# yukw777/EILEV

Hardware: AMD Instinct MI355X
Metric: clips/sec (8-frame, 16 in-context) encode+generate, eilev-blip2-opt-2.7b (higher is better)
Workload: dtype bf16

## Files before the change

### eilev_amd/csrc/gemm_pp4.h

```cpp
#pragma once
#include "gemm_common.h"

namespace {

#ifndef EILEV_PP4_DEEP
#define EILEV_PP4_DEEP 1
#endif
template <int EPI, bool F8 = false, int LN = 0, int M16K = 0, bool A3 = false>
__global__ __launch_bounds__(512, 2) void gemm_pp4_kernel(const GemmArgs g) {
    constexpr bool M16 = M16K != 0, HT16 = M16K == 2;
    static_assert(!M16 || !F8, "16 x 16 form: bf16 instances");
    constexpr int BM = 256, BN = 256, NWM = 2, NWN = 4, NW = 8;
    constexpr int WM = BM / NWM, WN = BN / NWN, TM = WM / 32, TN = WN / 32;
    constexpr int STEP = (BM + BN) * 128;
    constexpr int PC = 8;
    static_assert(!A3 || M16, "A3: lean epilogues only");
    constexpr int STG0 = A3 ? 2 * BM * 128 : 2 * STEP;

    extern __shared__ __attribute__((aligned(16))) char smem[];
    auto a_slot = [&](int st) { return smem + (A3 ? (st % 3) * (BM * 128) : (st & 1) * STEP); };
    auto w_slot = [&](int st) { return smem + (A3 ? 3 * (BM * 128) + (st & 1) * (BN * 128) : (st & 1) * STEP + BM * 128); };
    const int tiles_m = (g.M + BM - 1) / BM, tiles_n = (g.N + BN - 1) / BN, ntiles = tiles_m * tiles_n;
    const int tid = threadIdx.x, lane = tid & 63;
    const int wid = __builtin_amdgcn_readfirstlane(tid >> 6);
    const int wm = wid / NWN, wn = wid % NWN;
    const int l31 = lane & 31, hi = lane >> 5;
    const int l15 = lane & 15, g4 = lane >> 4;
    constexpr int TM16 = WM / 16, TN16 = WN / 16;
    const int ns = g.K / 64;
    const bool late = wid >= NW / 2;
    const int prow = lane >> 3, pslot = lane & 7;

    __amdgpu_buffer_rsrc_t ra = __builtin_amdgcn_make_buffer_rsrc((void *)g.A, 0, 0x7fffffff, 0x00020000);
    const __amdgpu_buffer_rsrc_t rw = __builtin_amdgcn_make_buffer_rsrc((void *)g.W, 0, 0x7fffffff, 0x00020000);
    unsigned po[PC];
    const int pw = late ? wid - NW / 2 : wid;
    auto set_tile = [&](int t, int &m0, int &n0) {
        int tm_i, tn_i;
        tile_coords(g, tiles_m, tiles_n, tm_i, tn_i, t);
        m0 = tm_i * BM;
        n0 = tn_i * BN;
        {
#ifdef EILEV_PP4_PROBE_A0
            const uint64_t base = (uint64_t)(g.A);
#else
            const uint64_t base = (uint64_t)(g.A + (int64_t)m0 * g.lda);
#endif
            const uint64_t ub = ((uint64_t)(unsigned)__builtin_amdgcn_readfirstlane((int)(base >> 32)) << 32) |
                                (unsigned)__builtin_amdgcn_readfirstlane((int)(unsigned)base);
            ra = __builtin_amdgcn_make_buffer_rsrc((void *)ub, 0, 0x7fffffff, 0x00020000);
        }
#pragma unroll
        for (int i = 0; i < PC; ++i) {
            const int row = (pw * PC + i) * 8 + prow;
            const unsigned sw = (unsigned)((pslot ^ ((row >> 1) & 7)) << 4);
            if (!late) {
                int gr = m0 + row;
                gr = gr < g.M ? gr : g.M - 1;
                po[i] = (unsigned)(gr - m0) * (unsigned)(g.lda * 2) + sw;
            } else {
                int gr = n0 + row;
                gr = gr < g.N ? gr : g.N - 1;
                po[i] = (unsigned)gr * (unsigned)(g.ldw * 2) + sw;
            }
        }
    };
    auto stage_step = [&](int st, bool mine = true, int part = 0) {
        char *sd = (late ? w_slot(st) : a_slot(st)) + (pw * PC) * 1024;
        if (!mine) return;
#ifndef EILEV_PP4_PROBE_SKIP
#define EILEV_PP4_PROBE_SKIP 0
#endif
        constexpr int PCE = (EILEV_PP4_PROBE_SKIP & 4) ? 0 : (EILEV_PP4_PROBE_SKIP & 1) ? PC / 2 : PC;
        constexpr int PCL = (EILEV_PP4_PROBE_SKIP & 8) ? 0 : (EILEV_PP4_PROBE_SKIP & 2) ? PC / 2 : PC;
        if (late) {
#pragma unroll
            for (int i = 0; i < PCL; ++i)
                if (part == 0 || (part == 1) == (i < PC / 2)) __builtin_amdgcn_raw_ptr_buffer_load_lds(rw, (lds_void *)(sd + i * 1024), 16, po[i], st * 128, 0, 0);
        } else {
#pragma unroll
            for (int i = 0; i < PCE; ++i)
                if (part == 0 || (part == 1) == (i < PC / 2)) __builtin_amdgcn_raw_ptr_buffer_load_lds(ra, (lds_void *)(sd + i * 1024), 16, po[i], st * 128, 0, 0);
        }
    };
    f32x16 acc[M16 ? 1 : TM][M16 ? 1 : TN];
    bf16x8 af[2][TM], bfr[2][TN];
    typedef __attribute__((ext_vector_type(4))) float f32x4_t;
    f32x4_t acc16[M16 ? TM16 : 1][M16 ? TN16 : 1];
    auto read_half = [&](int st, int h) {
        const char *sa = a_slot(st) + (wm * WM) * 128;
        const char *sb = w_slot(st) + (wn * WN) * 128;
        if constexpr (M16) {
            const int kc = h * 4 + g4;
#pragma unroll
            for (int j = 0; j < TN16; ++j) {
                const int row = j * 16 + l15;
                bfr[j >> 1][j & 1] = *reinterpret_cast<const bf16x8 *>(sb + row * 128 + swz(row, kc));
            }
#pragma unroll
            for (int i = 0; i < TM16; ++i) {
                const int row = i * 16 + l15;
                af[i >> 2][i & 3] = *reinterpret_cast<const bf16x8 *>(sa + row * 128 + swz(row, kc));
            }
            return;
        }
#pragma unroll
        for (int k2 = 0; k2 < 2; ++k2) {
            const int kc = h * 4 + k2 * 2 + hi;
#pragma unroll
            for (int j = 0; j < TN; ++j) {
                const int row = j * 32 + l31;
                bfr[k2][j] = *reinterpret_cast<const bf16x8 *>(sb + row * 128 + swz(row, kc));
            }
#pragma unroll
            for (int i = 0; i < TM; ++i) {
                const int row = i * 32 + l31;
                af[k2][i] = *reinterpret_cast<const bf16x8 *>(sa + row * 128 + swz(row, kc));
            }
        }
    };
    typedef int i32x8_t __attribute__((ext_vector_type(8)));
    struct Pair16 { bf16x8 lo, hi; };
    auto cat32 = [](const bf16x8 &lo, const bf16x8 &hi2) { return __builtin_bit_cast(i32x8_t, Pair16{lo, hi2}); };
    auto mma_half = [&]() {
        __builtin_amdgcn_s_setprio(1);
        if constexpr (F8) {
#pragma unroll
            for (int i = 0; i < TM; ++i)
#pragma unroll
                for (int j = 0; j < TN; ++j)
                    acc[i][j] = __builtin_amdgcn_mfma_scale_f32_32x32x64_f8f6f4(cat32(bfr[0][j], bfr[1][j]), cat32(af[0][i], af[1][i]), acc[i][j],
                                                                               0, 0, 0, 0, 0, 0);
        } else if constexpr (M16) {
#pragma unroll
            for (int i = 0; i < TM16; ++i)
#pragma unroll
                for (int j = 0; j < TN16; ++j)
                    acc16[i][j] = __builtin_amdgcn_mfma_f32_16x16x32_bf16(bfr[j >> 1][j & 1], af[i >> 2][i & 3], acc16[i][j], 0, 0, 0);
        } else {
#pragma unroll
            for (int k2 = 0; k2 < 2; ++k2)
#pragma unroll
                for (int i = 0; i < TM; ++i)
#pragma unroll
                    for (int j = 0; j < TN; ++j)
                        acc[i][j] = __builtin_amdgcn_mfma_f32_32x32x16_bf16(bfr[k2][j], af[k2][i], acc[i][j], 0, 0, 0);
        }
        __builtin_amdgcn_s_setprio(0);
    };
    const int hm = wm * 2 + (wn >> 1), hn = wn & 1;
    auto read_half_ht = [&](int st, int h) {
        const char *sa = a_slot(st) + (hm * 64) * 128;
        const char *sb = w_slot(st) + (hn * 64) * 128;
        if constexpr (M16) {
            const int kc = h * 4 + g4;
#pragma unroll
            for (int j = 0; j < 4; ++j) {
                const int row = j * 16 + l15;
                bfr[j >> 1][j & 1] = *reinterpret_cast<const bf16x8 *>(sb + row * 128 + swz(row, kc));
            }
#pragma unroll
            for (int i = 0; i < 4; ++i) {
                const int row = i * 16 + l15;
                af[0][i] = *reinterpret_cast<const bf16x8 *>(sa + row * 128 + swz(row, kc));
            }
            return;
        }
#pragma unroll
        for (int k2 = 0; k2 < 2; ++k2) {
            const int kc = h * 4 + k2 * 2 + hi;
#pragma unroll
            for (int j = 0; j < 2; ++j) {
                const int row = j * 32 + l31;
                bfr[k2][j] = *reinterpret_cast<const bf16x8 *>(sb + row * 128 + swz(row, kc));
            }
#pragma unroll
            for (int i = 0; i < 2; ++i) {
                const int row = i * 32 + l31;
                af[k2][i] = *reinterpret_cast<const bf16x8 *>(sa + row * 128 + swz(row, kc));
            }
        }
    };
    auto mma_half_ht = [&]() {
        __builtin_amdgcn_s_setprio(1);
        if constexpr (F8) {
#pragma unroll
            for (int i = 0; i < 2; ++i)
#pragma unroll
                for (int j = 0; j < 2; ++j)
                    acc[i][j] = __builtin_amdgcn_mfma_scale_f32_32x32x64_f8f6f4(cat32(bfr[0][j], bfr[1][j]), cat32(af[0][i], af[1][i]), acc[i][j],
                                                                               0, 0, 0, 0, 0, 0);
        } else if constexpr (M16) {
#pragma unroll
            for (int i = 0; i < 4; ++i)
#pragma unroll
                for (int j = 0; j < 4; ++j)
                    acc16[i][j] = __builtin_amdgcn_mfma_f32_16x16x32_bf16(bfr[j >> 1][j & 1], af[0][i], acc16[i][j], 0, 0, 0);
        } else {
#pragma unroll
            for (int k2 = 0; k2 < 2; ++k2)
#pragma unroll
                for (int i = 0; i < 2; ++i)
#pragma unroll
                    for (int j = 0; j < 2; ++j)
                        acc[i][j] = __builtin_amdgcn_mfma_f32_32x32x16_bf16(bfr[k2][j], af[k2][i], acc[i][j], 0, 0, 0);
        }
        __builtin_amdgcn_s_setprio(0);
    };
    char *const stg = smem + STG0 + wid * 4096;
    const unsigned stg_sw = (unsigned)(STG0 + wid * 4096 + l31 * 128 + hi * 8) ^ (unsigned)((l31 & 7) << 4);
    const unsigned stg_sw16 = (unsigned)(STG0 + wid * 4096 + l15 * 128 + (g4 & 1) * 8) ^ (unsigned)((((g4 >> 1) ^ (l15 & 7)) << 4));
    const int srow = lane >> 3, schunk = lane & 7;
    auto is_lean = [&](int n0_) {
        return !(n0_ + 128 >= g.N && !(g.dbg & DBG_GEMM_NO_HALF_TILES)) && n0_ + BN <= g.N && !g.out_f32 && g.patch_group == 0 && g.scale_cols == 0 && !g.wscale && !g.ascale &&
               !(g.dbg & (DBG_GEMM_NO_EPILOGUE | DBG_GEMM_NO_STORES | DBG_GEMM_ROW0_STORES)) && !(g.dbg & DBG_GEMM_PP4_NO_PRESTAGE);
    };
    float ln_rs[LN == 1 ? (M16 ? TM16 : TM) : 1];
    auto lean_epilogue = [&](int cm0, int cn0, auto res_c, auto ht_c) {
        constexpr bool RES = decltype(res_c)::value;
        constexpr bool HTE = decltype(ht_c)::value;
        constexpr int NU = HTE ? 2 : TM;
        const int roff = HTE ? hm * 64 : wm * WM, coff = HTE ? hn * 64 : wn * WN;
        if constexpr (M16K == 1) {
            if (cn0 + coff >= g.N) return;
        }
        constexpr bool LNC = LN == 1 && !RES, LNP = LN == 2 && RES;
        typedef __attribute__((ext_vector_type(4))) unsigned u32x4_t;
        const int r0 = cm0 + roff;
        const int rows = g.M - r0 < 0 ? 0 : (g.M - r0 < NU * 32 ? g.M - r0 : NU * 32);
        auto uniform_rsrc = [&](const void *ptr, int bytes) {
            const uint64_t base = (uint64_t)ptr;
            const uint64_t ub = ((uint64_t)(unsigned)__builtin_amdgcn_readfirstlane((int)(base >> 32)) << 32) |
                                (unsigned)__builtin_amdgcn_readfirstlane((int)(unsigned)base);
            return __builtin_amdgcn_make_buffer_rsrc((void *)ub, 0, __builtin_amdgcn_readfirstlane(bytes), 0x00020000);
        };
        const __amdgpu_buffer_rsrc_t rc = uniform_rsrc(reinterpret_cast<bf16 *>(g.C) + (int64_t)r0 * g.ldc + cn0 + coff, rows * (int)(g.ldc * 2));
        const __amdgpu_buffer_rsrc_t rr = uniform_rsrc(RES ? g.resid + (int64_t)r0 * g.ldr + cn0 + coff : g.A, RES ? rows * (int)(g.ldr * 2) : 0);
        const unsigned st_voff = (unsigned)srow * (unsigned)(g.ldc * 2) + schunk * 16, rs_voff = (unsigned)srow * (unsigned)(g.ldr * 2) + schunk * 16;
#ifndef EILEV_HM_AUX
#define EILEV_HM_AUX EILEV_ST_AUX
#endif
        constexpr bool HMI = LN == 1 && !RES && EPI == 0 && M16K == 1;
        const bool hm = HMI && g.hm_tok != 0;
        __amdgpu_buffer_rsrc_t rch = rc;
        unsigned hm_off = 0, hm_off_w = 0;
        int hm_str2 = 0, hm_t = 0;
        if constexpr (HMI) {
            if (hm) {
                const int TOK = g.hm_tok, HD = g.hm_hd, NH = g.hm_heads, D3 = g.N / 3;
                const int n0 = cn0 + coff;
                const int plane = __builtin_amdgcn_readfirstlane(n0 / D3), rr = n0 - plane * D3;
                int2 ent;
                if (rr < NH * 64) {
                    ent.x = (plane * NH + (rr >> 6)) * TOK * HD + schunk * 8;
                    ent.y = 64;
                } else {
                    const int cph = (HD - 64) >> 3, jb = ((rr - NH * 64) >> 3) + schunk, hh = jb / cph;
                    ent.x = (plane * NH + hh) * TOK * HD + TOK * 64 + (jb - hh * cph) * 8;
                    ent.y = HD - 64;
                }
                const int fw = __builtin_amdgcn_readfirstlane(r0 / TOK);
                const int m0 = r0 + srow, f0 = m0 / TOK;
                hm_t = m0 - f0 * TOK;
                hm_str2 = __builtin_amdgcn_readfirstlane(ent.y * 2);
                hm_off = (unsigned)(((f0 - fw) * TOK * g.N + ent.x + hm_t * ent.y) * 2);
                hm_off_w = hm_off + (unsigned)(TOK * g.N * 2) - (unsigned)(TOK * hm_str2);
                const int64_t left = ((int64_t)g.M / TOK - fw) * TOK * g.N * 2;
                rch = uniform_rsrc(reinterpret_cast<bf16 *>(g.C) + (int64_t)fw * TOK * g.N, (int)(unsigned)(left < 0xfffffff0ll ? left : 0xfffffff0ll));
            }
        }
        u32x4_t rv[4];
        auto res_load = [&](int u) {
#pragma unroll
            for (int it = 0; it < 4; ++it) rv[it] = __builtin_amdgcn_raw_buffer_load_b128(rr, rs_voff, (u * 32 + it * 8) * (int)(g.ldr * 2), 0);
        };
        if constexpr (RES) res_load(0);
        bf16x4 biasr[M16 ? 1 : TN][4];
        bf16x4 biasr16[M16 ? TN16 : 1];
        if constexpr (M16) {
#pragma unroll
            for (int j = 0; j < TN16; ++j) {
                if (g.bias) biasr16[j] = *reinterpret_cast<const bf16x4 *>(g.bias + cn0 + coff + j * 16 + g4 * 4);
                else biasr16[j] = (bf16x4){(bf16)0.f, (bf16)0.f, (bf16)0.f, (bf16)0.f};
            }
        } else {
#pragma unroll
        for (int j = 0; j < TN; ++j)
#pragma unroll
            for (int q = 0; q < 4; ++q) {
                if (g.bias) biasr[j][q] = *reinterpret_cast<const bf16x4 *>(g.bias + cn0 + wn * WN + j * 32 + q * 8 + hi * 4);
                else biasr[j][q] = (bf16x4){(bf16)0.f, (bf16)0.f, (bf16)0.f, (bf16)0.f};
            }
        }
        typedef __attribute__((ext_vector_type(2))) float f32x2_t;
        __amdgpu_buffer_rsrc_t rst = rr;
        if constexpr (LNP) rst = uniform_rsrc(g.stat_out + ((int64_t)((cn0 + coff) >> 6) * g.stat_ld + r0) * 2, rows * 8);
        static_for<NU>([&](auto u_c) {
            constexpr int U = decltype(u_c)::value;
            float st1 = 0.0f, st2 = 0.0f;
            bf16x4 rcell[M16 ? 2 : TN][4];
            if constexpr (RES) {
#pragma unroll
                for (int it = 0; it < 4; ++it) {
                    const int row = it * 8 + srow;
                    *reinterpret_cast<u32x4_t *>(stg + row * 128 + ((schunk ^ (row & 7)) << 4)) = rv[it];
                }
                if constexpr (U + 1 < NU) res_load(U + 1);
                if constexpr (M16) {
#pragma unroll
                    for (int ib = 0; ib < 2; ++ib)
#pragma unroll
                        for (int j = 0; j < TN16; ++j) {
                            unsigned ca;
                            asm volatile("v_xor_b32 %0, %1, %2" : "=v"(ca) : "n"(((j * 2) << 4) | (ib << 11)), "v"(stg_sw16));
                            rcell[ib][j] = *reinterpret_cast<const bf16x4 *>(smem + ca);
                        }
                } else {
#pragma unroll
                for (int j = 0; j < TN; ++j)
#pragma unroll
                    for (int q = 0; q < 4; ++q) {
                        unsigned ca;
                        asm volatile("v_xor_b32 %0, %1, %2" : "=v"(ca) : "n"((j * 4 + q) << 4), "v"(stg_sw));
                        rcell[j][q] = *reinterpret_cast<const bf16x4 *>(smem + ca);
                    }
                }
            }
            float st16[2][2] = {{0.0f, 0.0f}, {0.0f, 0.0f}};
            if constexpr (M16) {
#pragma unroll
                for (int ib = 0; ib < 2; ++ib)
#pragma unroll
                    for (int j = 0; j < TN16; ++j) {
                        float v[4];
                        if constexpr (LNC) {
#pragma unroll
                            for (int e = 0; e < 4; ++e) v[e] = fmaf(acc16[2 * U + ib][j][e], ln_rs[2 * U + ib], (float)biasr16[j][e]);
                        } else {
#pragma unroll
                            for (int e = 0; e < 4; ++e) v[e] = acc16[2 * U + ib][j][e] + (float)biasr16[j][e];
                        }
                        if constexpr (LN == 0 && EPI == 0 && !RES) {
                            if (cn0 + coff + j * 16 < g.scale_cols) {
#pragma unroll
                                for (int e = 0; e < 4; ++e) v[e] *= g.scale;
                            }
                        }
                        if constexpr (EPI == 2) {
#pragma unroll
                            for (int e = 0; e < 4; ++e) v[e] = fmaxf(v[e], 0.0f);
                        }
                        if constexpr (EPI == 1) gelu_erf_n<4>(v);
                        if constexpr (RES) {
#pragma unroll
                            for (int e = 0; e < 4; ++e) v[e] += (float)rcell[ib][j][e];
                        }
                        if constexpr (LNP) {
#pragma unroll
                            for (int e = 0; e < 4; ++e) {
                                st16[ib][0] += v[e];
                                st16[ib][1] = fmaf(v[e], v[e], st16[ib][1]);
                            }
                        }
                        unsigned ca;
                        asm volatile("v_xor_b32 %0, %1, %2" : "=v"(ca) : "n"(((j * 2) << 4) | (ib << 11)), "v"(stg_sw16));
                        *reinterpret_cast<bf16x4 *>(smem + ca) = (bf16x4){(bf16)v[0], (bf16)v[1], (bf16)v[2], (bf16)v[3]};
                    }
            } else {
#pragma unroll
            for (int j = 0; j < TN; ++j)
#pragma unroll
                for (int q = 0; q < 4; ++q) {
                    float v[4];
                    if constexpr (LNC) {
#pragma unroll
                        for (int e = 0; e < 4; ++e) v[e] = fmaf(acc[U][j][q * 4 + e], ln_rs[U], (float)biasr[j][q][e]);
                    } else {
#pragma unroll
                        for (int e = 0; e < 4; ++e) v[e] = acc[U][j][q * 4 + e] + (float)biasr[j][q][e];
                    }
                    if constexpr (EPI == 2) {
#pragma unroll
                        for (int e = 0; e < 4; ++e) v[e] = fmaxf(v[e], 0.0f);
                    }
                    if constexpr (EPI == 1) gelu_erf_n<4>(v);
                    if constexpr (RES) {
#pragma unroll
                        for (int e = 0; e < 4; ++e) v[e] += (float)rcell[j][q][e];
                    }
                    if constexpr (LNP) {
#pragma unroll
                        for (int e = 0; e < 4; ++e) {
                            st1 += v[e];
                            st2 = fmaf(v[e], v[e], st2);
                        }
                    }
                    unsigned ca;
                    asm volatile("v_xor_b32 %0, %1, %2" : "=v"(ca) : "n"((j * 4 + q) << 4), "v"(stg_sw));
                    *reinterpret_cast<bf16x4 *>(smem + ca) = (bf16x4){(bf16)v[0], (bf16)v[1], (bf16)v[2], (bf16)v[3]};
                }
            }
            if constexpr (LNP && M16) {
                typedef __attribute__((ext_vector_type(2))) unsigned u32x2_t;
#pragma unroll
                for (int ib = 0; ib < 2; ++ib) {
                    float a1 = st16[ib][0], a2 = st16[ib][1];
                    a1 += __shfl_xor(a1, 16); a2 += __shfl_xor(a2, 16);
                    a1 += __shfl_xor(a1, 32); a2 += __shfl_xor(a2, 32);
                    const f32x2_t t = (f32x2_t){a1, a2};
                    if (g4 == 0) __builtin_amdgcn_raw_buffer_store_b64(__builtin_bit_cast(u32x2_t, t), rst, (U * 32 + ib * 16 + l15) * 8, 0, 0);
                }
            } else if constexpr (LNP) {
                typedef __attribute__((ext_vector_type(2))) unsigned u32x2_t;
                const f32x2_t t = (f32x2_t){st1 + __shfl_xor(st1, 32), st2 + __shfl_xor(st2, 32)};
                if (hi == 0) __builtin_amdgcn_raw_buffer_store_b64(__builtin_bit_cast(u32x2_t, t), rst, (U * 32 + l31) * 8, 0, 0);
            }
            __builtin_amdgcn_sched_barrier(0);
            bf16x8 erb[2];
#pragma unroll
            for (int h2 = 0; h2 < 2; ++h2) {
#pragma unroll
                for (int b = 0; b < 2; ++b) {
                    const int row = (h2 * 2 + b) * 8 + srow;
                    erb[b] = *reinterpret_cast<const bf16x8 *>(stg + row * 128 + ((schunk ^ (row & 7)) << 4));
                }
                if (hm) {
                    if constexpr (HMI) {
#pragma unroll
                        for (int b = 0; b < 2; ++b) {
                            const int RO = U * 32 + (h2 * 2 + b) * 8;
                            const unsigned vo = hm_t + RO >= g.hm_tok ? hm_off_w : hm_off;
                            __builtin_amdgcn_raw_buffer_store_b128(__builtin_bit_cast(u32x4_t, erb[b]), rch, vo, RO * hm_str2, EILEV_HM_AUX);
                        }
                    }
                } else {
#pragma unroll
                for (int b = 0; b < 2; ++b)
                    __builtin_amdgcn_raw_buffer_store_b128(__builtin_bit_cast(u32x4_t, erb[b]), rc, st_voff, (U * 32 + (h2 * 2 + b) * 8) * (int)(g.ldc * 2), EILEV_ST_AUX);
                }
            }
            asm volatile("s_nop 1" ::: "memory");
            __builtin_amdgcn_sched_barrier(0);
        });
    };
#define PP_WAIT_LGKM0() __builtin_amdgcn_s_waitcnt(0xC07F)
#define PP_WAIT_LGKM0_VM0() __builtin_amdgcn_s_waitcnt(0x0070)
#define PP_WAIT_VM0() __builtin_amdgcn_s_waitcnt(0x0F70)
#define PP_BARRIER()                       \
    do {                                   \
        __builtin_amdgcn_sched_barrier(0); \
        __builtin_amdgcn_s_barrier();      \
        __builtin_amdgcn_sched_barrier(0); \
    } while (0)

    int t = blockIdx.x, m0, n0;
    if (t >= ntiles) return;
    set_tile(t, m0, n0);
    auto w_piece_mine = [&](int n0_) { return !(n0_ + 128 >= g.N && !(g.dbg & DBG_GEMM_NO_HALF_TILES)) || wid < NW / 2 + 2; };
    stage_step(0, w_piece_mine(n0));
    bool pre1 = ns > 1 && (A3 || !(g.dbg & DBG_GEMM_PP4_NO_PRESTAGE));
    if (pre1) stage_step(1, w_piece_mine(n0));
    bool lean_cur = M16 || is_lean(n0);
    float ln_nm[LN == 1 ? (M16 ? TM16 : TM) : 1], ln_cl[LN == 1 ? (M16 ? TN16 : TN) : 1];
    auto ln_fetch = [&](int m0_, int n0_) {
        if constexpr (LN == 1 && M16) {
            const bool ht = HT16 && n0_ + 128 >= g.N;
            const int mb = m0_ + (ht ? hm * 64 : wm * WM) + l15, nb = n0_ + (ht ? hn * 64 : wn * WN) + l15;
            const __amdgpu_buffer_rsrc_t rl = __builtin_amdgcn_make_buffer_rsrc((void *)g.ln_rows, 0, g.M * 8, 0x00020000);
            const __amdgpu_buffer_rsrc_t rcs = __builtin_amdgcn_make_buffer_rsrc((void *)g.ln_csum, 0, g.N * 4, 0x00020000);
#pragma unroll
            for (int i = 0; i < TM16; ++i) ln_nm[i] = __builtin_bit_cast(float, __builtin_amdgcn_raw_buffer_load_b32(rl, (mb + i * 16) * 8 + 4, 0, 0));
#pragma unroll
            for (int j = 0; j < TN16; ++j) ln_cl[j] = __builtin_bit_cast(float, __builtin_amdgcn_raw_buffer_load_b32(rcs, (nb + j * 16) * 4, 0, 0));
        } else if constexpr (LN == 1) {
            const bool ht = n0_ + 128 >= g.N && !(g.dbg & DBG_GEMM_NO_HALF_TILES);
            const int mb = m0_ + (ht ? hm * 64 : wm * WM) + l31, nb = n0_ + (ht ? hn * 64 : wn * WN) + l31;
            const __amdgpu_buffer_rsrc_t rl = __builtin_amdgcn_make_buffer_rsrc((void *)g.ln_rows, 0, g.M * 8, 0x00020000);
            const __amdgpu_buffer_rsrc_t rcs = __builtin_amdgcn_make_buffer_rsrc((void *)g.ln_csum, 0, g.N * 4, 0x00020000);
#pragma unroll
            for (int i = 0; i < TM; ++i) ln_nm[i] = __builtin_bit_cast(float, __builtin_amdgcn_raw_buffer_load_b32(rl, (mb + i * 32) * 8 + 4, 0, 0));
#pragma unroll
            for (int j = 0; j < TN; ++j) ln_cl[j] = __builtin_bit_cast(float, __builtin_amdgcn_raw_buffer_load_b32(rcs, (nb + j * 32) * 4, 0, 0));
        }
    };
    ln_fetch(m0, n0);
    int trace_i = 0;
    const bool tracer = g.trace != nullptr && (wid == 0 || wid == NW / 2) && lane == 0;
#ifdef EILEV_PP4_ITRACE
#define ITR(k)                                                                                                              \
    do {                                                                                                                    \
        if (st == EILEV_PP4_ITRACE && tracer) *reinterpret_cast<volatile unsigned long long *>(stg + (k) * 8) = __builtin_amdgcn_s_memtime(); \
    } while (0)
#else
#define ITR(k) do { } while (0)
#endif
    auto stamp = [&](int k, bool core = false) {
#ifdef EILEV_PP4_ITRACE
        return;
#endif
        if (tracer && trace_i < g.trace_tiles)
            g.trace[(((size_t)blockIdx.x * 2 + (late ? 1 : 0)) * g.trace_tiles + trace_i) * 8 + k] =
                core ? __builtin_amdgcn_s_memtime() : __builtin_amdgcn_s_memrealtime();
    };
    for (; t < ntiles; t += gridDim.x) {
        stamp(0);
        stamp(5, true);
        typedef __attribute__((ext_vector_type(4))) short s16x4_t;
        s16x4_t ln_a1[LN == 1 ? (M16 ? TM16 : TM) : 1], ln_w1[LN == 1 ? (M16 ? TN16 : TN) : 1];
        auto acc_prep = [&]() {
            if constexpr (LN == 1 && M16) {
                const bf16 z = (bf16)0.0f;
#pragma unroll
                for (int i = 0; i < TM16; ++i) {
                    const float m = g4 ? 0.0f : ln_nm[i];
                    const bf16 mh = (bf16)m, ml = (bf16)(m - (float)mh);
                    ln_a1[i] = __builtin_bit_cast(s16x4_t, (bf16x4){mh, mh, ml, z});
                }
#pragma unroll
                for (int j = 0; j < TN16; ++j) {
                    const float c = g4 ? 0.0f : ln_cl[j];
                    const bf16 ch = (bf16)c, cl = (bf16)(c - (float)ch);
                    ln_w1[j] = __builtin_bit_cast(s16x4_t, (bf16x4){ch, cl, ch, z});
                }
            } else if constexpr (LN == 1) {
                const bf16 z = (bf16)0.0f;
#pragma unroll
                for (int i = 0; i < TM; ++i) {
                    const float m = hi ? 0.0f : ln_nm[i];
                    const bf16 mh = (bf16)m, ml = (bf16)(m - (float)mh);
                    ln_a1[i] = __builtin_bit_cast(s16x4_t, (bf16x4){mh, mh, ml, z});
                }
#pragma unroll
                for (int j = 0; j < TN; ++j) {
                    const float c = hi ? 0.0f : ln_cl[j];
                    const bf16 ch = (bf16)c, cl = (bf16)(c - (float)ch);
                    ln_w1[j] = __builtin_bit_cast(s16x4_t, (bf16x4){ch, cl, ch, z});
                }
            }
        };
        auto acc_init = [&]() {
            if constexpr (M16) {
                const f32x4_t zero4 = (f32x4_t){0.0f, 0.0f, 0.0f, 0.0f};
#pragma unroll
                for (int i = 0; i < TM16; ++i)
#pragma unroll
                    for (int j = 0; j < TN16; ++j) {
                        if constexpr (LN == 1) acc16[i][j] = __builtin_amdgcn_mfma_f32_16x16x16bf16_1k(ln_w1[j], ln_a1[i], zero4, 0, 0, 0);
                        else acc16[i][j] = zero4;
                    }
            } else if constexpr (LN == 1) {
                f32x16 zero;
#pragma unroll
                for (int r = 0; r < 16; ++r) zero[r] = 0.0f;
#pragma unroll
                for (int i = 0; i < TM; ++i)
#pragma unroll
                    for (int j = 0; j < TN; ++j) acc[i][j] = __builtin_amdgcn_mfma_f32_32x32x8bf16_1k(ln_w1[j], ln_a1[i], zero, 0, 0, 0);
            } else {
#pragma unroll
                for (int i = 0; i < TM; ++i)
#pragma unroll
                    for (int j = 0; j < TN; ++j)
#pragma unroll
                        for (int r = 0; r < 16; ++r) acc[i][j][r] = 0.0f;
            }
        };
        if constexpr (LN != 1) acc_init();
        asm volatile("s_waitcnt vmcnt(0)" ::: "memory");
        PP_BARRIER();
        if (late) PP_BARRIER();
        stamp(1);
        const int nsd = (g.dbg & DBG_GEMM_ONE_KSTEP) ? 1 : ns;
        const bool half_tile = n0 + 128 >= g.N && !(g.dbg & DBG_GEMM_NO_HALF_TILES);
        auto kstep = [&](int st, auto first_c, auto ht_c) {
            constexpr bool FIRST = decltype(first_c)::value;
            constexpr bool HT = decltype(ht_c)::value;
            const bool w_mine = !HT || wid < NW / 2 + 2;
            ITR(0);
            if constexpr (HT) read_half_ht(st, 0); else read_half(st, 0);
#if EILEV_PP4_DEEP
#ifndef EILEV_PP4_SPLIT
#define EILEV_PP4_SPLIT 3
#endif
#ifndef EILEV_PP4_SPLIT_QKV
#define EILEV_PP4_SPLIT_QKV 0
#endif
            constexpr bool SPLIT_OK = !HT && (EILEV_PP4_SPLIT_QKV || !(LN == 1 && EPI == 0));
            constexpr bool SPLIT_E = (EILEV_PP4_SPLIT & 1) && SPLIT_OK, SPLIT_L = (EILEV_PP4_SPLIT & 2) && SPLIT_OK;
            if (!late) {
                if constexpr (A3) {
                    if (st + 2 < ns) stage_step(st + 2, w_mine, SPLIT_E ? 1 : 0);
                } else if (st + 1 < ns && !(FIRST && pre1)) stage_step(st + 1, w_mine, SPLIT_E ? 1 : 0);
            } else if (FIRST && !pre1 && ns > 1) stage_step(1, w_mine);
            else if (SPLIT_L && !FIRST && st + 1 < ns) stage_step(st + 1, w_mine, 2);
#else
            if (st + 1 < ns && !(FIRST && pre1)) stage_step(st + 1, w_mine);
#endif
            if constexpr (FIRST && LN == 1) acc_prep();
            PP_WAIT_LGKM0();
            ITR(1);
            PP_BARRIER();
            ITR(2);
            if constexpr (FIRST && LN == 1) acc_init();
            if constexpr (HT) mma_half_ht(); else mma_half();
            ITR(3);
            PP_BARRIER();
            ITR(4);
            if constexpr (HT) read_half_ht(st, 1); else read_half(st, 1);
#if EILEV_PP4_DEEP
            PP_WAIT_LGKM0();
            if (late) {
                PP_WAIT_VM0();
                if constexpr (!HT) if (st + 2 < ns) stage_step(st + 2, w_mine, SPLIT_L ? 1 : 0);
            } else if (A3) {
                if (SPLIT_E && st + 2 < ns) stage_step(st + 2, w_mine, 2);
            } else if (SPLIT_E && st + 1 < ns && !(FIRST && pre1)) stage_step(st + 1, w_mine, 2);
            ITR(5);
            PP_BARRIER();
            ITR(6);
            if constexpr (HT) {
                if (late && st + 2 < ns) stage_step(st + 2, w_mine);
                mma_half_ht();
            } else mma_half();
            __builtin_amdgcn_sched_barrier(0);
            if constexpr (A3) {
                if (!late) {
                    if (st + 2 < ns) asm volatile("s_waitcnt vmcnt(8)" ::: "memory");
                    else asm volatile("s_waitcnt vmcnt(0)" ::: "memory");
                }
            } else if (!late) asm volatile("s_waitcnt vmcnt(0)" ::: "memory");
            ITR(7);
            PP_BARRIER();
#else
            PP_WAIT_LGKM0_VM0();
            PP_BARRIER();
            if constexpr (HT) mma_half_ht(); else mma_half();
            PP_BARRIER();
#endif
        };
        if (half_tile && M16K != 1) {
            if constexpr (M16K != 1) {
                kstep(0, std::true_type{}, std::true_type{});
                for (int st = 1; st < nsd; ++st) kstep(st, std::false_type{}, std::true_type{});
            }
        } else {
            kstep(0, std::true_type{}, std::false_type{});
            for (int st = 1; st < nsd; ++st) kstep(st, std::false_type{}, std::false_type{});
        }
        stamp(2);
#ifdef EILEV_PP4_ITRACE
        if (tracer && trace_i < g.trace_tiles) {
#pragma unroll
            for (int k = 0; k < 8; ++k)
                g.trace[(((size_t)blockIdx.x * 2 + (late ? 1 : 0)) * g.trace_tiles + trace_i) * 8 + k] = *reinterpret_cast<volatile unsigned long long *>(stg + k * 8);
        }
#endif
        if (!late) PP_BARRIER();
        if constexpr (LN == 1) {
            const __amdgpu_buffer_rsrc_t rl = __builtin_amdgcn_make_buffer_rsrc((void *)g.ln_rows, 0, g.M * 8, 0x00020000);
            if constexpr (M16) {
#pragma unroll
                for (int i = 0; i < TM16; ++i) ln_rs[i] = __builtin_bit_cast(float, __builtin_amdgcn_raw_buffer_load_b32(rl, (m0 + ((HT16 && half_tile) ? hm * 64 : wm * WM) + i * 16 + l15) * 8, 0, 0));
            } else {
#pragma unroll
            for (int u = 0; u < TM; ++u) ln_rs[u] = __builtin_bit_cast(float, __builtin_amdgcn_raw_buffer_load_b32(rl, (m0 + wm * WM + u * 32 + l31) * 8, 0, 0));
            }
        }
        const int cm0 = m0, cn0 = n0, tn = t + gridDim.x;
        const bool lean = lean_cur;
        pre1 = false;
        lean_cur = false;
        if (tn < ntiles) {
            set_tile(tn, m0, n0);
            stage_step(0, w_piece_mine(n0));
            pre1 = lean && ns > 1;
            if (pre1) stage_step(1, w_piece_mine(n0));
            lean_cur = M16 || is_lean(n0);
            ln_fetch(m0, n0);
        }
        stamp(3);
        if (HT16 && half_tile) {
            if constexpr (HT16) {
                if constexpr (LN == 1) lean_epilogue(cm0, cn0, std::false_type{}, std::true_type{});
                else if constexpr (LN == 2) lean_epilogue(cm0, cn0, std::true_type{}, std::true_type{});
                else if (g.resid != nullptr) lean_epilogue(cm0, cn0, std::true_type{}, std::true_type{});
                else lean_epilogue(cm0, cn0, std::false_type{}, std::true_type{});
            }
        } else if (lean || M16) {
            if constexpr (LN == 1) lean_epilogue(cm0, cn0, std::false_type{}, std::false_type{});
            else if constexpr (LN == 2) lean_epilogue(cm0, cn0, std::true_type{}, std::false_type{});
            else if (g.resid != nullptr) lean_epilogue(cm0, cn0, std::true_type{}, std::false_type{});
            else lean_epilogue(cm0, cn0, std::false_type{}, std::false_type{});
        } else if constexpr (!M16) {
            if (half_tile) {
                gemm_epilogue<64, 64, EPI, 0, 2, LN, true>(g, reinterpret_cast<f32x16(&)[2][2]>(acc), smem + STEP, cm0, cn0, hm, hn, wid, lane);
            } else {
                gemm_epilogue<WM, WN, EPI, 0, TM / 2, LN, true>(g, acc, smem + STEP, cm0, cn0, wm, wn, wid, lane);
                gemm_epilogue<WM, WN, EPI, TM / 2, TM, LN, true>(g, acc, smem + STEP, cm0, cn0, wm, wn, wid, lane);
            }
        }
        stamp(4);
        stamp(6, true);
        ++trace_i;
    }
#undef PP_BARRIER
}

constexpr int PP4_SMEM = 2 * 65536 + 8 * 4096;

}
```

Measured before the change: 229.2.

## Prefetch epilogue bias/residual/LN loads early and use partial vmcnt waits in pp4 GEMM

```diff
diff --git a/eilev_amd/csrc/gemm_pp4.h b/eilev_amd/csrc/gemm_pp4.h
--- a/eilev_amd/csrc/gemm_pp4.h
+++ b/eilev_amd/csrc/gemm_pp4.h
@@ -215,14 +215,112 @@
         return !(n0_ + 128 >= g.N && !(g.dbg & DBG_GEMM_NO_HALF_TILES)) && n0_ + BN <= g.N && !g.out_f32 && g.patch_group == 0 && g.scale_cols == 0 && !g.wscale && !g.ascale &&
                !(g.dbg & (DBG_GEMM_NO_EPILOGUE | DBG_GEMM_NO_STORES | DBG_GEMM_ROW0_STORES)) && !(g.dbg & DBG_GEMM_PP4_NO_PRESTAGE);
     };
+    float ln_nm[LN == 1 ? (M16 ? TM16 : TM) : 1], ln_cl[LN == 1 ? (M16 ? TN16 : TN) : 1];
+    int trace_i = 0;
+    const bool tracer = g.trace != nullptr && (wid == 0 || wid == NW / 2) && lane == 0;
+    auto stamp = [&](int k, bool core = false) {
+#ifdef EILEV_PP4_ITRACE
+        return;
+#endif
+        if (tracer && trace_i < g.trace_tiles)
+            g.trace[(((size_t)blockIdx.x * 2 + (late ? 1 : 0)) * g.trace_tiles + trace_i) * 8 + k] =
+                core ? __builtin_amdgcn_s_memtime() : __builtin_amdgcn_s_memrealtime();
+    };
     float ln_rs[LN == 1 ? (M16 ? TM16 : TM) : 1];
-    auto lean_epilogue = [&](int cm0, int cn0, auto res_c, auto ht_c) {
+    typedef __attribute__((ext_vector_type(2))) unsigned u32x2_e;
+    typedef __attribute__((ext_vector_type(4))) unsigned u32x4_e;
+    u32x2_e ep_bias[M16 ? TN16 : 1];
+#ifndef EILEV_PP4_RES_UNITS
+#define EILEV_PP4_RES_UNITS 1
+#endif
+    constexpr int EP_RU = EILEV_PP4_RES_UNITS;
+    static_assert(EP_RU == 1 || EP_RU == 2, "residual units in front of the DMA");
+    u32x4_e ep_rv[M16 ? EP_RU : 1][4];
+    int ep_young = 0;
+#define PP_ASM_LOAD4(op, step, first, d0, d1, d2, d3, voff, rsrc)                                                                              \
+    asm volatile("s_nop 4\n\t" op " %0, %4, %5, 0 offen offset:%6\n\t" op " %1, %4, %5, 0 offen offset:%7\n\t" op " %2, %4, %5, 0 offen offset:%8\n\t" op \
+                 " %3, %4, %5, 0 offen offset:%9"                                                                                             \
+                 : "=&v"(d0), "=&v"(d1), "=&v"(d2), "=&v"(d3)                                                                                 \
+                 : "v"(voff), "s"(rsrc), "n"(first), "n"((first) + (step)), "n"((first) + 2 * (step)), "n"((first) + 3 * (step)))
+#define PP_ASM_LOAD4_B128(d0, d1, d2, d3, voff, rsrc, s0, s1, s2, s3)                                                                              \
+    asm volatile("s_nop 4\n\tbuffer_load_dwordx4 %0, %4, %5, %6 offen\n\tbuffer_load_dwordx4 %1, %4, %5, %7 offen\n\tbuffer_load_dwordx4 %2, %4, %5, %8 " \
+                 "offen\n\tbuffer_load_dwordx4 %3, %4, %5, %9 offen"                                                                                \
+                 : "=&v"(d0), "=&v"(d1), "=&v"(d2), "=&v"(d3)                                                                                     \
+                 : "v"(voff), "s"(rsrc), "s"(s0), "s"(s1), "s"(s2), "s"(s3))
+    auto epi_block = [&](bool ht, int &roff, int &coff) {
+        roff = (HT16 && ht) ? hm * 64 : wm * WM;
+        coff = (HT16 && ht) ? hn * 64 : wn * WN;
+    };
+    auto epi_res = [&]() { return LN == 2 || (LN == 0 && g.resid != nullptr); };
+    auto epi_rr = [&](int cm0, int cn0, bool ht, int nu) {
+        int roff, coff;
+        epi_block(ht, roff, coff);
+        const int r0 = cm0 + roff;
+        const int rows = (g.M - r0 < 0 || !epi_res()) ? 0 : (g.M - r0 < nu * 32 ? g.M - r0 : nu * 32);
+        const uint64_t base = (uint64_t)(g.resid + (int64_t)r0 * g.ldr + cn0 + coff);
+        const uint64_t ub = ((uint64_t)(unsigned)__builtin_amdgcn_readfirstlane((int)(base >> 32)) << 32) | (unsigned)__builtin_amdgcn_readfirstlane((int)(unsigned)base);
+        return __builtin_amdgcn_make_buffer_rsrc((void *)ub, 0, __builtin_amdgcn_readfirstlane(rows * (int)(g.ldr * 2)), 0x00020000);
+    };
+    auto epi_issue = [&](int cm0, int cn0, bool ht) {
+        if constexpr (M16) {
+            int roff, coff;
+            epi_block(ht, roff, coff);
+            if constexpr (LN == 1) {
+                const __amdgpu_buffer_rsrc_t rl = __builtin_amdgcn_make_buffer_rsrc((void *)g.ln_rows, 0, g.M * 8, 0x00020000);
+                const unsigned vo = (unsigned)(cm0 + roff + l15) * 8u;
+                static_assert(TM16 == 8 && TN16 == 4, "the grouped asm loads below");
+                PP_ASM_LOAD4("buffer_load_dword", 128, 0, ln_rs[0], ln_rs[1], ln_rs[2], ln_rs[3], vo, rl);
+                PP_ASM_LOAD4("buffer_load_dword", 128, 512, ln_rs[4], ln_rs[5], ln_rs[6], ln_rs[7], vo, rl);
+            }
+            {
+                const __amdgpu_buffer_rsrc_t rb = __builtin_amdgcn_make_buffer_rsrc((void *)g.bias, 0, g.bias ? g.N * 2 : 0, 0x00020000);
+                const unsigned vo = (unsigned)(cn0 + coff + g4 * 4) * 2u;
+                PP_ASM_LOAD4("buffer_load_dwordx2", 32, 0, ep_bias[0], ep_bias[1], ep_bias[2], ep_bias[3], vo, rb);
+            }
+            if constexpr (LN != 1) {
+                const __amdgpu_buffer_rsrc_t rr = epi_rr(cm0, cn0, ht, (HT16 && ht) ? 2 : TM);
+                const unsigned vo = (unsigned)srow * (unsigned)(g.ldr * 2) + schunk * 16;
+                const int rs8 = 8 * (int)(g.ldr * 2);
+#pragma unroll
+                for (int u = 0; u < EP_RU; ++u) PP_ASM_LOAD4_B128(ep_rv[u][0], ep_rv[u][1], ep_rv[u][2], ep_rv[u][3], vo, rr, (4 * u) * rs8, (4 * u + 1) * rs8, (4 * u + 2) * rs8, (4 * u + 3) * rs8);
+            }
+        }
+    };
+    auto epi_wait = [&]() {
+        if constexpr (M16) {
+            const int ny = __builtin_amdgcn_readfirstlane(ep_young);
+#define PP_EPI_WAIT_ASM "s_cmp_lt_u32 %[ny], 16\n\ts_cbranch_scc1 1f\n\ts_waitcnt vmcnt(16)\n\ts_branch 3f\n1:\n\ts_cmp_lt_u32 %[ny], 8\n\ts_cbranch_scc1 2f\n\ts_waitcnt vmcnt(8)\n\ts_branch 3f\n2:\n\ts_waitcnt vmcnt(0)\n3:"
+            if constexpr (LN == 1) {
+                asm volatile(PP_EPI_WAIT_ASM
+                             : "+v"(ep_bias[0]), "+v"(ep_bias[1]), "+v"(ep_bias[2]), "+v"(ep_bias[3]), "+v"(ln_rs[0]), "+v"(ln_rs[1]), "+v"(ln_rs[2]), "+v"(ln_rs[3]),
+                               "+v"(ln_rs[4]), "+v"(ln_rs[5]), "+v"(ln_rs[6]), "+v"(ln_rs[7])
+                             : [ny] "s"(ny)
+                             : "memory", "scc");
+                asm volatile("" : "+v"(ln_nm[0]), "+v"(ln_nm[1]), "+v"(ln_nm[2]), "+v"(ln_nm[3]), "+v"(ln_nm[4]), "+v"(ln_nm[5]), "+v"(ln_nm[6]), "+v"(ln_nm[7]),
+                                  "+v"(ln_cl[0]), "+v"(ln_cl[1]), "+v"(ln_cl[2]), "+v"(ln_cl[3]));
+            } else if constexpr (EP_RU == 2) {
+                asm volatile(PP_EPI_WAIT_ASM
+                             : "+v"(ep_bias[0]), "+v"(ep_bias[1]), "+v"(ep_bias[2]), "+v"(ep_bias[3]), "+v"(ep_rv[0][0]), "+v"(ep_rv[0][1]), "+v"(ep_rv[0][2]),
+                               "+v"(ep_rv[0][3]), "+v"(ep_rv[EP_RU - 1][0]), "+v"(ep_rv[EP_RU - 1][1]), "+v"(ep_rv[EP_RU - 1][2]), "+v"(ep_rv[EP_RU - 1][3])
+                             : [ny] "s"(ny)
+                             : "memory", "scc");
+            } else {
+                asm volatile(PP_EPI_WAIT_ASM
+                             : "+v"(ep_bias[0]), "+v"(ep_bias[1]), "+v"(ep_bias[2]), "+v"(ep_bias[3]), "+v"(ep_rv[0][0]), "+v"(ep_rv[0][1]), "+v"(ep_rv[0][2]),
+                               "+v"(ep_rv[0][3])
+                             : [ny] "s"(ny)
+                             : "memory", "scc");
+            }
+#undef PP_EPI_WAIT_ASM
+        }
+    };
+    auto lean_epilogue = [&](int cm0, int cn0, auto res_c, auto ht_c) -> int {
         constexpr bool RES = decltype(res_c)::value;
         constexpr bool HTE = decltype(ht_c)::value;
         constexpr int NU = HTE ? 2 : TM;
         const int roff = HTE ? hm * 64 : wm * WM, coff = HTE ? hn * 64 : wn * WN;
         if constexpr (M16K == 1) {
-            if (cn0 + coff >= g.N) return;
+            if (cn0 + coff >= g.N) return 0;
         }
         constexpr bool LNC = LN == 1 && !RES, LNP = LN == 2 && RES;
         typedef __attribute__((ext_vector_type(4))) unsigned u32x4_t;
@@ -248,6 +346,9 @@
         if constexpr (HMI) {
             if (hm) {
                 const int TOK = g.hm_tok, HD = g.hm_hd, NH = g.hm_heads, D3 = g.N / 3;
+                int zero_o = 0;
+                asm volatile("" : "+v"(zero_o));
+                const int schunk = (int)__builtin_amdgcn_mbcnt_hi(~0u, __builtin_amdgcn_mbcnt_lo(~0u, (unsigned)zero_o)) & 7;
                 const int n0 = cn0 + coff;
                 const int plane = __builtin_amdgcn_readfirstlane(n0 / D3), rr = n0 - plane * D3;
                 int2 ent;
@@ -255,7 +356,9 @@
                     ent.x = (plane * NH + (rr >> 6)) * TOK * HD + schunk * 8;
                     ent.y = 64;
                 } else {
-                    const int cph = (HD - 64) >> 3, jb = ((rr - NH * 64) >> 3) + schunk, hh = jb / cph;
+                    const int cph = (HD - 64) >> 3, jb = ((rr - NH * 64) >> 3) + schunk;
+                    const unsigned mg = (unsigned)__builtin_amdgcn_readfirstlane((int)(0xffffffffu / (unsigned)cph + 1u));
+                    const int hh = cph == 1 ? jb : (int)__umulhi((unsigned)jb, mg);
                     ent.x = (plane * NH + hh) * TOK * HD + TOK * 64 + (jb - hh * cph) * 8;
                     ent.y = HD - 64;
                 }
@@ -274,15 +377,12 @@
 #pragma unroll
             for (int it = 0; it < 4; ++it) rv[it] = __builtin_amdgcn_raw_buffer_load_b128(rr, rs_voff, (u * 32 + it * 8) * (int)(g.ldr * 2), 0);
         };
-        if constexpr (RES) res_load(0);
+        if constexpr (RES && !M16) res_load(0);
         bf16x4 biasr[M16 ? 1 : TN][4];
         bf16x4 biasr16[M16 ? TN16 : 1];
         if constexpr (M16) {
 #pragma unroll
-            for (int j = 0; j < TN16; ++j) {
-                if (g.bias) biasr16[j] = *reinterpret_cast<const bf16x4 *>(g.bias + cn0 + coff + j * 16 + g4 * 4);
-                else biasr16[j] = (bf16x4){(bf16)0.f, (bf16)0.f, (bf16)0.f, (bf16)0.f};
-            }
+            for (int j = 0; j < TN16; ++j) biasr16[j] = __builtin_bit_cast(bf16x4, ep_bias[j]);
         } else {
 #pragma unroll
         for (int j = 0; j < TN; ++j)
@@ -303,9 +403,16 @@
 #pragma unroll
                 for (int it = 0; it < 4; ++it) {
                     const int row = it * 8 + srow;
-                    *reinterpret_cast<u32x4_t *>(stg + row * 128 + ((schunk ^ (row & 7)) << 4)) = rv[it];
-                }
-                if constexpr (U + 1 < NU) res_load(U + 1);
+                    if constexpr (M16) *reinterpret_cast<u32x4_t *>(stg + row * 128 + ((schunk ^ (row & 7)) << 4)) = __builtin_bit_cast(u32x4_t, ep_rv[U % EP_RU][it]);
+                    else *reinterpret_cast<u32x4_t *>(stg + row * 128 + ((schunk ^ (row & 7)) << 4)) = rv[it];
+                }
+                if constexpr (M16) {
+                    if constexpr (U + EP_RU < NU) {
+#pragma unroll
+                        for (int it = 0; it < 4; ++it)
+                            ep_rv[U % EP_RU][it] = __builtin_bit_cast(u32x4_e, __builtin_amdgcn_raw_buffer_load_b128(rr, rs_voff, ((U + EP_RU) * 32 + it * 8) * (int)(g.ldr * 2), 0));
+                    }
+                } else if constexpr (U + 1 < NU) res_load(U + 1);
                 if constexpr (M16) {
 #pragma unroll
                     for (int ib = 0; ib < 2; ++ib)
@@ -442,6 +549,7 @@
             asm volatile("s_nop 1" ::: "memory");
             __builtin_amdgcn_sched_barrier(0);
         });
+        return NU * 4 + (LNP && M16 ? NU * 2 : 0) + (RES && M16 ? (NU - EP_RU) * 4 : 0);
     };
 #define PP_WAIT_LGKM0() __builtin_amdgcn_s_waitcnt(0xC07F)
 #define PP_WAIT_LGKM0_VM0() __builtin_amdgcn_s_waitcnt(0x0070)
@@ -457,21 +565,18 @@
     if (t >= ntiles) return;
     set_tile(t, m0, n0);
     auto w_piece_mine = [&](int n0_) { return !(n0_ + 128 >= g.N && !(g.dbg & DBG_GEMM_NO_HALF_TILES)) || wid < NW / 2 + 2; };
-    stage_step(0, w_piece_mine(n0));
     bool pre1 = ns > 1 && (A3 || !(g.dbg & DBG_GEMM_PP4_NO_PRESTAGE));
-    if (pre1) stage_step(1, w_piece_mine(n0));
     bool lean_cur = M16 || is_lean(n0);
-    float ln_nm[LN == 1 ? (M16 ? TM16 : TM) : 1], ln_cl[LN == 1 ? (M16 ? TN16 : TN) : 1];
     auto ln_fetch = [&](int m0_, int n0_) {
         if constexpr (LN == 1 && M16) {
             const bool ht = HT16 && n0_ + 128 >= g.N;
             const int mb = m0_ + (ht ? hm * 64 : wm * WM) + l15, nb = n0_ + (ht ? hn * 64 : wn * WN) + l15;
             const __amdgpu_buffer_rsrc_t rl = __builtin_amdgcn_make_buffer_rsrc((void *)g.ln_rows, 0, g.M * 8, 0x00020000);
             const __amdgpu_buffer_rsrc_t rcs = __builtin_amdgcn_make_buffer_rsrc((void *)g.ln_csum, 0, g.N * 4, 0x00020000);
-#pragma unroll
-            for (int i = 0; i < TM16; ++i) ln_nm[i] = __builtin_bit_cast(float, __builtin_amdgcn_raw_buffer_load_b32(rl, (mb + i * 16) * 8 + 4, 0, 0));
-#pragma unroll
-            for (int j = 0; j < TN16; ++j) ln_cl[j] = __builtin_bit_cast(float, __builtin_amdgcn_raw_buffer_load_b32(rcs, (nb + j * 16) * 4, 0, 0));
+            const unsigned vm = (unsigned)mb * 8u, vn = (unsigned)nb * 4u;
+            PP_ASM_LOAD4("buffer_load_dword", 128, 4, ln_nm[0], ln_nm[1], ln_nm[2], ln_nm[3], vm, rl);
+            PP_ASM_LOAD4("buffer_load_dword", 128, 516, ln_nm[4], ln_nm[5], ln_nm[6], ln_nm[7], vm, rl);
+            PP_ASM_LOAD4("buffer_load_dword", 64, 0, ln_cl[0], ln_cl[1], ln_cl[2], ln_cl[3], vn, rcs);
         } else if constexpr (LN == 1) {
             const bool ht = n0_ + 128 >= g.N && !(g.dbg & DBG_GEMM_NO_HALF_TILES);
             const int mb = m0_ + (ht ? hm * 64 : wm * WM) + l31, nb = n0_ + (ht ? hn * 64 : wn * WN) + l31;
@@ -483,9 +588,21 @@
             for (int j = 0; j < TN; ++j) ln_cl[j] = __builtin_bit_cast(float, __builtin_amdgcn_raw_buffer_load_b32(rcs, (nb + j * 32) * 4, 0, 0));
         }
     };
-    ln_fetch(m0, n0);
-    int trace_i = 0;
-    const bool tracer = g.trace != nullptr && (wid == 0 || wid == NW / 2) && lane == 0;
+    int head_young = 0;
+    if constexpr (M16) {
+        ln_fetch(m0, n0);
+        stage_step(0, w_piece_mine(n0));
+        if (pre1) stage_step(1, w_piece_mine(n0));
+        if constexpr (LN == 1) {
+            asm volatile("s_waitcnt vmcnt(0)"
+                         : "+v"(ln_nm[0]), "+v"(ln_nm[1]), "+v"(ln_nm[2]), "+v"(ln_nm[3]), "+v"(ln_nm[4]), "+v"(ln_nm[5]), "+v"(ln_nm[6]), "+v"(ln_nm[7]),
+                           "+v"(ln_cl[0]), "+v"(ln_cl[1]), "+v"(ln_cl[2]), "+v"(ln_cl[3])::"memory");
+        } else head_young = pre1 && w_piece_mine(n0) && !EILEV_PP4_PROBE_SKIP ? PC : 0;
+    } else {
+        stage_step(0, w_piece_mine(n0));
+        if (pre1) stage_step(1, w_piece_mine(n0));
+        ln_fetch(m0, n0);
+    }
 #ifdef EILEV_PP4_ITRACE
 #define ITR(k)                                                                                                              \
     do {                                                                                                                    \
@@ -494,14 +611,6 @@
 #else
 #define ITR(k) do { } while (0)
 #endif
-    auto stamp = [&](int k, bool core = false) {
-#ifdef EILEV_PP4_ITRACE
-        return;
-#endif
-        if (tracer && trace_i < g.trace_tiles)
-            g.trace[(((size_t)blockIdx.x * 2 + (late ? 1 : 0)) * g.trace_tiles + trace_i) * 8 + k] =
-                core ? __builtin_amdgcn_s_memtime() : __builtin_amdgcn_s_memrealtime();
-    };
     for (; t < ntiles; t += gridDim.x) {
         stamp(0);
         stamp(5, true);
@@ -566,7 +675,17 @@
             }
         };
         if constexpr (LN != 1) acc_init();
-        asm volatile("s_waitcnt vmcnt(0)" ::: "memory");
+        if constexpr (M16) {
+            const int hy = __builtin_amdgcn_readfirstlane(head_young);
+            if (hy >= 40) asm volatile("s_waitcnt vmcnt(40)" ::: "memory");
+            else if (hy >= 32) asm volatile("s_waitcnt vmcnt(32)" ::: "memory");
+            else if (hy >= 24) asm volatile("s_waitcnt vmcnt(24)" ::: "memory");
+            else if (hy >= 16) asm volatile("s_waitcnt vmcnt(16)" ::: "memory");
+            else if (hy >= 8) asm volatile("s_waitcnt vmcnt(8)" ::: "memory");
+            else asm volatile("s_waitcnt vmcnt(0)" ::: "memory");
+        } else {
+            asm volatile("s_waitcnt vmcnt(0)" ::: "memory");
+        }
         PP_BARRIER();
         if (late) PP_BARRIER();
         stamp(1);
@@ -656,7 +775,8 @@
         }
 #endif
         if (!late) PP_BARRIER();
-        if constexpr (LN == 1) {
+        if constexpr (M16) epi_issue(m0, n0, half_tile);
+        if constexpr (LN == 1 && !M16) {
             const __amdgpu_buffer_rsrc_t rl = __builtin_amdgcn_make_buffer_rsrc((void *)g.ln_rows, 0, g.M * 8, 0x00020000);
             if constexpr (M16) {
 #pragma unroll
@@ -670,27 +790,33 @@
         const bool lean = lean_cur;
         pre1 = false;
         lean_cur = false;
+        ep_young = 0;
         if (tn < ntiles) {
             set_tile(tn, m0, n0);
+            if constexpr (M16) ln_fetch(m0, n0);
             stage_step(0, w_piece_mine(n0));
             pre1 = lean && ns > 1;
             if (pre1) stage_step(1, w_piece_mine(n0));
             lean_cur = M16 || is_lean(n0);
-            ln_fetch(m0, n0);
-        }
+            if constexpr (!M16) ln_fetch(m0, n0);
+            if (w_piece_mine(n0) && !EILEV_PP4_PROBE_SKIP) ep_young = pre1 ? 2 * PC : PC;
+        }
+        head_young = ep_young >= 2 * PC ? PC : 0;
         stamp(3);
+        epi_wait();
+        if constexpr (M16) stamp(7);
         if (HT16 && half_tile) {
             if constexpr (HT16) {
-                if constexpr (LN == 1) lean_epilogue(cm0, cn0, std::false_type{}, std::true_type{});
-                else if constexpr (LN == 2) lean_epilogue(cm0, cn0, std::true_type{}, std::true_type{});
-                else if (g.resid != nullptr) lean_epilogue(cm0, cn0, std::true_type{}, std::true_type{});
-                else lean_epilogue(cm0, cn0, std::false_type{}, std::true_type{});
+                if constexpr (LN == 1) head_young += lean_epilogue(cm0, cn0, std::false_type{}, std::true_type{});
+                else if constexpr (LN == 2) head_young += lean_epilogue(cm0, cn0, std::true_type{}, std::true_type{});
+                else if (g.resid != nullptr) head_young += lean_epilogue(cm0, cn0, std::true_type{}, std::true_type{});
+                else head_young += lean_epilogue(cm0, cn0, std::false_type{}, std::true_type{});
             }
         } else if (lean || M16) {
-            if constexpr (LN == 1) lean_epilogue(cm0, cn0, std::false_type{}, std::false_type{});
-            else if constexpr (LN == 2) lean_epilogue(cm0, cn0, std::true_type{}, std::false_type{});
-            else if (g.resid != nullptr) lean_epilogue(cm0, cn0, std::true_type{}, std::false_type{});
-            else lean_epilogue(cm0, cn0, std::false_type{}, std::false_type{});
+            if constexpr (LN == 1) head_young += lean_epilogue(cm0, cn0, std::false_type{}, std::false_type{});
+            else if constexpr (LN == 2) head_young += lean_epilogue(cm0, cn0, std::true_type{}, std::false_type{});
+            else if (g.resid != nullptr) head_young += lean_epilogue(cm0, cn0, std::true_type{}, std::false_type{});
+            else head_young += lean_epilogue(cm0, cn0, std::false_type{}, std::false_type{});
         } else if constexpr (!M16) {
             if (half_tile) {
                 gemm_epilogue<64, 64, EPI, 0, 2, LN, true>(g, reinterpret_cast<f32x16(&)[2][2]>(acc), smem + STEP, cm0, cn0, hm, hn, wid, lane);
```

Result: no change. 231.3, median of 6 (+0.9%).
